# sanweiliti/RoHM

Hardware: AMD Instinct MI355X
Metric: denoised 145-frame clips/sec @1000 DDPM steps (higher is better)
Workload: dtype f32

## Files before the change

rohm_amd/csrc/encoder_chain.hip:

```cpp
#include <type_traits>
#include "common.h"
#include "gemm_sched.h"
#include "attention_tile.h"

namespace rohm {

typedef float f32x16c __attribute__((ext_vector_type(16)));

namespace chain {

constexpr int BM = 144, BK = kGemmBK, NRB = BM / 16;
constexpr int A_UNITS = BM * 8, A_ITERS = (A_UNITS + 255) / 256;
constexpr int kMaxBN = 384;
constexpr int kZone = 2 * (BM + kMaxBN) * BK;
constexpr int kLdsFloats = kZone + 512 + 4 * BM * 2;
constexpr int kSc1 = 16;

struct PhaseArgs {
    const float* A; int lda;
    const float* W; int ldw;
    float* C; int ldc;
    int K;
    const float* bias;
    const float* R; int ldr;
    const float* gamma; const float* beta; float eps; int ln_dim;
    int qcols; float qscale;
    int S; const float* tab; const float* tab0; int ldtab, ldtab0, tab_by_row;
    int m0, n0;
    float* row_stats; unsigned tag28; int tn, tiles_n;
    unsigned* err; unsigned xcc1; int fault;
};

__device__ __forceinline__ int head_row(int n0, int t) { return ((t % 96) >> 5) * 512 + n0 + (t / 96) * 32 + (t & 31); }

template <int BN, bool HEAD = false>
__device__ __forceinline__ void prefetch_w(const float* W, int ldw, int n0, float* smem, int tid, int wave_u) {
    constexpr int B_ITERS = BN * 8 / 256;
    float* Bs = smem + 2 * BM * BK;
#pragma unroll
    for (int buf = 0; buf < 2; ++buf)
#pragma unroll
        for (int i = 0; i < B_ITERS; ++i) {
            const int u = tid + i * 256;
            const int row = u >> 3;
            const int slot = (u & 7) ^ ((row >> 1) & 7);
            const float* src = W + (size_t)(HEAD ? head_row(n0, row) : n0 + row) * ldw + slot * 4 + buf * BK;
            __builtin_amdgcn_global_load_lds((const __attribute__((address_space(1))) void*)src,
                                             (__attribute__((address_space(3))) void*)(Bs + buf * (BN * BK) + (i * 256 + wave_u) * 4), 16, 0, 0);
        }
}

__device__ __forceinline__ void group_sync(unsigned long long* flags, int tn, int G, unsigned tag, unsigned xcc1, unsigned* err, int tid) {
    asm volatile("s_waitcnt vmcnt(0)" ::: "memory");
    __syncthreads();
    if (tid == 0) {
        flags[tn] = ((unsigned long long)xcc1 << 32) | tag;
        asm volatile("" ::: "memory");
    }
    if (tid < G && tid != tn) {
        for (int it = 0;; ++it) {
            const unsigned long long f = __hip_atomic_load(flags + tid, __ATOMIC_RELAXED, __HIP_MEMORY_SCOPE_AGENT);
            if ((unsigned)f == tag && (f >> 32) != 0ull) {
                if ((unsigned)(f >> 32) != xcc1) __hip_atomic_store(err, 2u, __ATOMIC_RELAXED, __HIP_MEMORY_SCOPE_AGENT);
                break;
            }
            __builtin_amdgcn_s_sleep(1);
            if ((it & 127) == 127 && __hip_atomic_load(err, __ATOMIC_RELAXED, __HIP_MEMORY_SCOPE_AGENT) != 0u) break;
            if (it > (1 << 19)) {
                __hip_atomic_store(err, 1u, __ATOMIC_RELAXED, __HIP_MEMORY_SCOPE_AGENT);
                break;
            }
        }
    }
    __syncthreads();
}

template <int BN, int EPI, bool PREF, bool SC1, bool REFETCH, bool HEAD = false, typename AfterLoop>
__device__ __forceinline__ void gemm_phase(const PhaseArgs& p, float* smem, const int tid, AfterLoop&& after_loop,
                                           AtQFrags<2>* q_out = nullptr) {
    static_assert(EPI == EPI_BIAS_RES_LN || EPI == EPI_BIAS_GELU || EPI == EPI_QKV || EPI == EPI_EMBED, "chain phases: LN tail, GELU, QKV, embed");
    static_assert(!HEAD || (EPI == EPI_QKV && BN == 3 * AT_DH), "the head-aligned tile is one head's q | k | v");
    constexpr int WN = BN / 4;
    constexpr int NCB = WN / 16;
    constexpr int B_ITERS = BN * 8 / 256;
    constexpr int PIECES = A_ITERS + B_ITERS;
    constexpr int AUX = SC1 ? kSc1 : 0;

    float* As = smem;
    float* Bs = smem + 2 * BM * BK;
    float* lds_dummy = smem + kZone;
    float* const zone = lds_dummy + 512;
    float* const colrow = HEAD ? smem + 2 * AT_TILE : zone;
    static_assert(!HEAD || 2 * AT_TILE + 512 <= AT_LDS_FLOATS, "head-aligned tile: the bias row overruns the stack's LDS");

    const int lane = tid & 63;
    const int wave = tid >> 6;
    const int li = lane & 15, lg = lane >> 4;
    const int wave_u = __builtin_amdgcn_readfirstlane(wave) * 64;
    const int m0 = p.m0, n0 = p.n0;

    const float* a_src[A_ITERS];
#pragma unroll
    for (int i = 0; i < A_ITERS; ++i) {
        const int u = tid + i * 256;
        const int row = (u < A_UNITS) ? (u >> 3) : 0;
        const int slot = (u & 7) ^ ((row >> 1) & 7);
        a_src[i] = p.A + (size_t)(m0 + row) * p.lda + slot * 4;
    }
    const float* b_src[B_ITERS];
#pragma unroll
    for (int i = 0; i < B_ITERS; ++i) {
        const int u = tid + i * 256;
        const int row = u >> 3;
        const int slot = (u & 7) ^ ((row >> 1) & 7);
        b_src[i] = p.W + (size_t)(HEAD ? head_row(n0, row) : n0 + row) * p.ldw + slot * 4;
    }
    auto dma_a = [&](int buf, int k0) {
#pragma unroll
        for (int piece = 0; piece < A_ITERS; ++piece) {
            float* dst = As + buf * (BM * BK) + (piece * 256 + wave_u) * 4;
            if (piece == A_ITERS - 1 && A_UNITS % 256 != 0)
                dst = (wave_u < A_UNITS - (A_ITERS - 1) * 256) ? dst : lds_dummy + (wave_u & 64) * 4;
            __builtin_amdgcn_global_load_lds((const __attribute__((address_space(1))) void*)(a_src[piece] + k0),
                                             (__attribute__((address_space(3))) void*)dst, 16, 0, AUX);
        }
    };
    auto dma_b = [&](int buf, int k0) {
#pragma unroll
        for (int i = 0; i < B_ITERS; ++i)
            __builtin_amdgcn_global_load_lds((const __attribute__((address_space(1))) void*)(b_src[i] + k0),
                                             (__attribute__((address_space(3))) void*)(Bs + buf * (BN * BK) + (i * 256 + wave_u) * 4), 16, 0, 0);
    };

    f32x4 acc16[NRB * NCB];
#pragma unroll
    for (int i = 0; i < NRB * NCB; ++i) acc16[i] = f32x4{0.f, 0.f, 0.f, 0.f};
    constexpr int READS = NRB + NCB;
    constexpr int MFMAS = 4 * NRB * NCB;
    struct Frag { f32x4 a[NRB]; f32x4 b[NCB]; };
    Frag f0, f1;
    auto read_frags = [&](Frag& f, int buf, int ks) {
        const float* as = As + buf * (BM * BK);
        const float* bs = Bs + buf * (BN * BK) + wave * WN * BK;
        const int slot = ks * 4 + lg;
#pragma unroll
        for (int c = 0; c < NCB; ++c) f.b[c] = *reinterpret_cast<const f32x4*>(bs + lds_off(c * 16 + li, slot));
#pragma unroll
        for (int r = 0; r < NRB; ++r) f.a[r] = *reinterpret_cast<const f32x4*>(as + lds_off(r * 16 + li, slot));
    };
    auto mma_half = [&](const Frag& f) {
#pragma unroll
        for (int r = 0; r < NRB; ++r)
#pragma unroll
            for (int c = 0; c < NCB; ++c)
#pragma unroll
                for (int j = 0; j < 4; ++j)
                    acc16[r * NCB + c] = __builtin_amdgcn_mfma_f32_16x16x4f32(f.b[c][j], f.a[r][j], acc16[r * NCB + c], 0, 0, 0);
    };

    const int nk = p.K / BK;
    constexpr bool COL_LDS = BN >= 384;
    if constexpr (!PREF) { dma_b(0, 0); dma_b(1, BK); }
    if constexpr (COL_LDS) {
        if (wave == 0) {
#pragma unroll
            for (int h = 0; h < 2; ++h) {
                const int unit = h * 64 + lane;
                const int t = (unit < BN / 4 ? unit : BN / 4 - 1) * 4;
                const float* src = HEAD ? p.bias + head_row(n0, t) : p.bias + n0 + t;
                __builtin_amdgcn_global_load_lds((const __attribute__((address_space(1))) void*)src,
                                                 (__attribute__((address_space(3))) void*)(colrow + h * 256), 16, 0, 0);
            }
        }
    }
    dma_a(0, 0);
    dma_a(1, BK);

    const int nw = n0 + wave * WN;
    struct ColOps { f32x4 bias, g4, b4; };
    constexpr bool RES = (EPI == EPI_BIAS_RES_LN);
    constexpr bool HAS_RES = RES || EPI == EPI_EMBED;
    constexpr bool PEEL = BN <= 256;
    constexpr bool EARLY = PEEL && !COL_LDS;
    const f32x4 zero4 = f32x4{0.f, 0.f, 0.f, 0.f};
    auto load_col = [&](int nb) __attribute__((always_inline)) {
        ColOps o{zero4, zero4, zero4};
        if constexpr (EPI == EPI_EMBED) {  }
        else if constexpr (COL_LDS) o.bias = *reinterpret_cast<const f32x4*>(colrow + (nb - n0));
        else o.bias = *reinterpret_cast<const f32x4*>(p.bias + nb);
        if constexpr (RES) {
            o.g4 = *reinterpret_cast<const f32x4*>(p.gamma + nb);
            o.b4 = *reinterpret_cast<const f32x4*>(p.beta + nb);
        }
        return o;
    };
    auto for_units = [&](auto&& fn) __attribute__((always_inline)) {
#pragma unroll
        for (int r = 0; r < NRB; ++r)
#pragma unroll
            for (int c = 0; c < NCB; ++c) fn(c * NRB + r, c, m0 + r * 16 + li, nw + c * 16 + lg * 4, acc16[r * NCB + c]);
    };
    ColOps col[NCB];
    f32x4 res[HAS_RES ? NCB * NRB : 1];
    auto request_ops = [&]() __attribute__((always_inline)) {
#pragma unroll
        for (int c = 0; c < NCB; ++c) col[c] = load_col(nw + c * 16 + lg * 4);
        if constexpr (RES)
            for_units([&](int i, int, int m, int nb, f32x4) __attribute__((always_inline)) {
                res[i] = *reinterpret_cast<const f32x4*>(p.R + (size_t)m * p.ldr + nb);
            });
        if constexpr (EPI == EPI_EMBED)
            for_units([&](int i, int, int m, int nb, f32x4) __attribute__((always_inline)) {
                const int bidx = m / p.S, tok = m % p.S;
                const float* tp = (tok == 0) ? p.tab0 + (size_t)bidx * p.ldtab0 + nb : p.tab + (size_t)(p.tab_by_row ? m : tok) * p.ldtab + nb;
                res[i] = *reinterpret_cast<const f32x4*>(tp);
            });
    };

    asm volatile("s_waitcnt vmcnt(%0)" ::"n"(A_ITERS) : "memory");
    __syncthreads();
    read_frags(f0, 0, 0);
    constexpr int NG = READS;
    constexpr int MF = (MFMAS + NG - 1) / NG;
    auto chunk = [&](int kc, auto last_tag, auto dma_tag) __attribute__((always_inline)) {
        constexpr bool LAST = decltype(last_tag)::value;
        constexpr bool DMA = decltype(dma_tag)::value;
        const int buf = kc & 1;
        if constexpr (LAST && EARLY) request_ops();
        read_frags(f1, buf, 1);
        mma_half(f0);
        SchedGroups<0, NG, MF, READS, 0, 0>::run();
        __builtin_amdgcn_sched_barrier(0);
        if constexpr (!LAST) {
            asm volatile("s_waitcnt vmcnt(0)" ::: "memory");
            __syncthreads();
            __builtin_amdgcn_sched_barrier(0);
            if constexpr (DMA) {
                const int kn = ((kc + 2 < nk) ? (kc + 2) : (nk - 1)) * BK;
                dma_a(buf, kn);
                dma_b(buf, kn);
            }
            read_frags(f0, buf ^ 1, 0);
            mma_half(f1);
            SchedGroups<0, NG, MF, READS, DMA ? PIECES : 0, 1>::run();
        } else {
            mma_half(f1);
        }
        __builtin_amdgcn_sched_barrier(0);
    };
    using DmaTail = std::integral_constant<bool, REFETCH>;
    if constexpr (PEEL) {
        for (int kc = 0; kc + 2 < nk; ++kc) chunk(kc, std::false_type{}, std::true_type{});
        chunk(nk - 2, std::false_type{}, DmaTail{});
        chunk(nk - 1, std::true_type{}, std::false_type{});
    } else {
        for (int kc = 0; kc + 2 < nk; ++kc) chunk(kc, std::false_type{}, std::true_type{});
        chunk(nk - 2, std::false_type{}, DmaTail{});
        chunk(nk - 1, std::false_type{}, DmaTail{});
    }
    asm volatile("s_waitcnt vmcnt(0)" ::: "memory");
    __syncthreads();
    after_loop();
    if constexpr (!EARLY) request_ops();

    if constexpr (EPI == EPI_BIAS_RES_LN) {
#pragma unroll
        for (int c = 0; c < NCB; ++c)
#pragma unroll
            for (int r = 0; r < NRB; ++r) {
                f32x4& a = acc16[r * NCB + c];
                const f32x4 rr = res[c * NRB + r];
#pragma unroll
                for (int q = 0; q < 4; ++q) a[q] = (a[q] + col[c].bias[q]) + rr[q];
            }
        typedef unsigned rohm_u2 __attribute__((ext_vector_type(2)));
        auto merge_swap = [](float& m, float& q2, float n, bool far) __attribute__((always_inline)) {
            rohm_u2 tm, tq;
            if (far) { tm = __builtin_amdgcn_permlane32_swap(__float_as_uint(m), __float_as_uint(m), false, false);
                       tq = __builtin_amdgcn_permlane32_swap(__float_as_uint(q2), __float_as_uint(q2), false, false); }
            else     { tm = __builtin_amdgcn_permlane16_swap(__float_as_uint(m), __float_as_uint(m), false, false);
                       tq = __builtin_amdgcn_permlane16_swap(__float_as_uint(q2), __float_as_uint(q2), false, false); }
            const float ma = __uint_as_float(tm[0]), mb = __uint_as_float(tm[1]);
            const float d = mb - ma;
            m = 0.5f * (ma + mb);
            q2 = (__uint_as_float(tq[0]) + __uint_as_float(tq[1])) + 0.5f * n * d * d;
        };
        float* const part = zone;
        constexpr float kLane = (float)(4 * NCB);
#pragma unroll
        for (int r = 0; r < NRB; ++r) {
            float sm = 0.f;
#pragma unroll
            for (int c = 0; c < NCB; ++c)
#pragma unroll
                for (int k = 0; k < 4; ++k) sm += acc16[r * NCB + c][k];
            float m = sm * (1.0f / kLane), q2 = 0.f;
#pragma unroll
            for (int c = 0; c < NCB; ++c)
#pragma unroll
                for (int k = 0; k < 4; ++k) { const float d = acc16[r * NCB + c][k] - m; q2 += d * d; }
            merge_swap(m, q2, kLane, true);
            merge_swap(m, q2, 2.0f * kLane, false);
            if (lg == 0) *reinterpret_cast<f32x2*>(part + (wave * BM + r * 16 + li) * 2) = f32x2{m, q2};
        }
        __syncthreads();
        const int tn = p.tn, tiles_n = p.tiles_n;
        const unsigned xcc1 = p.xcc1, ep28 = p.tag28;
        const unsigned tag = (ep28 << 4) | xcc1;
        float* const row_stats = p.row_stats;
        if (tid < BM) {
            auto merge = [](float ma, float qa, float mb, float qb, float n, float& m, float& q2) __attribute__((always_inline)) {
                const float d = mb - ma;
                m = 0.5f * (ma + mb);
                q2 = (qa + qb) + 0.5f * n * d * d;
            };
            f32x2 w4[4];
#pragma unroll
            for (int w = 0; w < 4; ++w) w4[w] = *reinterpret_cast<const f32x2*>(part + (w * BM + tid) * 2);
            float m01, q01, m23, q23, a, b;
            merge(w4[0][0], w4[0][1], w4[1][0], w4[1][1], (float)WN, m01, q01);
            merge(w4[2][0], w4[2][1], w4[3][0], w4[3][1], (float)WN, m23, q23);
            merge(m01, q01, m23, q23, 2.0f * (float)WN, a, b);
            const unsigned pub = (p.fault && tn == 0) ? (tag ^ 0x80000000u) : tag;
            *reinterpret_cast<f32x4*>(row_stats + ((size_t)tn * BM + tid) * 4) = f32x4{a, __uint_as_float(pub), b, __uint_as_float(pub)};
            float mk[8], qk[8];
            for (int it = 0;; ++it) {
                unsigned long long lo[8], hi[8];
#pragma unroll
                for (int k = 0; k < 8; ++k) {
                    lo[k] = hi[k] = 0ull;
                    if (k < tiles_n && k != tn) {
                        const unsigned long long* sp = reinterpret_cast<const unsigned long long*>(row_stats + ((size_t)k * BM + tid) * 4);
                        lo[k] = __hip_atomic_load(sp, __ATOMIC_RELAXED, __HIP_MEMORY_SCOPE_AGENT);
                        hi[k] = __hip_atomic_load(sp + 1, __ATOMIC_RELAXED, __HIP_MEMORY_SCOPE_AGENT);
                    }
                }
                bool ok = true, same_xcd = true;
#pragma unroll
                for (int k = 0; k < 8; ++k) {
                    mk[k] = 0.f; qk[k] = 0.f;
                    if (k >= tiles_n) continue;
                    if (k == tn) { mk[k] = a; qk[k] = b; continue; }
                    const unsigned tl = (unsigned)(lo[k] >> 32), th = (unsigned)(hi[k] >> 32);
                    ok = ok && (tl >> 4) == ep28 && (th >> 4) == ep28 && (tl & 15u) != 0u && (th & 15u) != 0u;
                    same_xcd = same_xcd && (tl & 15u) == xcc1 && (th & 15u) == xcc1;
                    mk[k] = __uint_as_float((unsigned)lo[k]);
                    qk[k] = __uint_as_float((unsigned)hi[k]);
                }
                if (ok) {
                    if (!same_xcd) __hip_atomic_store(p.err, 2u, __ATOMIC_RELAXED, __HIP_MEMORY_SCOPE_AGENT);
                    break;
                }
                __builtin_amdgcn_s_sleep(1);
                if ((it & 127) == 127 && __hip_atomic_load(p.err, __ATOMIC_RELAXED, __HIP_MEMORY_SCOPE_AGENT) != 0u) break;
                if (it > (1 << 19)) {
                    __hip_atomic_store(p.err, 1u, __ATOMIC_RELAXED, __HIP_MEMORY_SCOPE_AGENT);
                    break;
                }
            }
            constexpr float kT = (float)BN;
            if (tiles_n > 1) {
                merge(mk[0], qk[0], mk[1], qk[1], kT, mk[0], qk[0]);
                if (tiles_n > 2) merge(mk[2], qk[2], mk[3], qk[3], kT, mk[2], qk[2]);
                if (tiles_n > 4) { merge(mk[4], qk[4], mk[5], qk[5], kT, mk[4], qk[4]); merge(mk[6], qk[6], mk[7], qk[7], kT, mk[6], qk[6]); }
            }
            if (tiles_n > 2) {
                merge(mk[0], qk[0], mk[2], qk[2], 2.0f * kT, mk[0], qk[0]);
                if (tiles_n > 4) merge(mk[4], qk[4], mk[6], qk[6], 2.0f * kT, mk[4], qk[4]);
            }
            if (tiles_n > 4) merge(mk[0], qk[0], mk[4], qk[4], 4.0f * kT, mk[0], qk[0]);
            const float mu = mk[0];
            const float var = qk[0] / (float)p.ln_dim;
            *reinterpret_cast<f32x2*>(part + tid * 2) = f32x2{mu, 1.0f / sqrtf(var + p.eps)};
        }
        __syncthreads();
#pragma unroll
        for (int r = 0; r < NRB; ++r) {
            const f32x2 mrv = *reinterpret_cast<const f32x2*>(part + (r * 16 + li) * 2);
#pragma unroll
            for (int c = 0; c < NCB; ++c) {
                const f32x4 a = acc16[r * NCB + c];
                f32x4 v;
#pragma unroll
                for (int q = 0; q < 4; ++q) v[q] = (a[q] - mrv[0]) * mrv[1] * col[c].g4[q] + col[c].b4[q];
                *reinterpret_cast<f32x4*>(p.C + (size_t)(m0 + r * 16 + li) * p.ldc + nw + c * 16 + lg * 4) = v;
            }
        }
    } else if constexpr (HEAD) {
        float* const Ks = smem;
        float* const Vs = smem + AT_TILE;
        auto put = [&](float* img, int c) __attribute__((always_inline)) {
            const int u = wave * 8 + (c & 1) * 4 + lg;
#pragma unroll
            for (int r = 0; r < NRB; ++r) {
                const f32x4 a = acc16[r * NCB + c];
                f32x4 v;
#pragma unroll
                for (int q = 0; q < 4; ++q) v[q] = a[q] + col[c].bias[q];
                if (c < 2) {
#pragma unroll
                    for (int q = 0; q < 4; ++q) v[q] *= p.qscale;
                }
                *reinterpret_cast<f32x4*>(img + (r * 16 + li) * AT_DH + ((u ^ li) << 2)) = v;
            }
        };
        put(Vs, 0); put(Vs, 1);
        put(Ks, 2); put(Ks, 3);
        __syncthreads();
#pragma unroll
        for (int ks = 0; ks < 8; ++ks) {
            const int sw = ((ks * 4 + lg) ^ li) << 2;
#pragma unroll
            for (int ps = 0; ps < 2; ++ps) q_out->f[ps][ks] = *reinterpret_cast<const f32x4*>(Vs + ((ps * 4 + wave) * 16 + li) * AT_DH + sw);
            q_out->c[ks] = *reinterpret_cast<const f32x4*>(Vs + (8 * 16 + li) * AT_DH + sw);
        }
        __syncthreads();
        put(Vs, 4); put(Vs, 5);
    } else if constexpr (EPI == EPI_EMBED) {
        for_units([&](int i, int, int m, int nb, f32x4 a) __attribute__((always_inline)) {
            const int tok = m % p.S;
            f32x4 v;
#pragma unroll
            for (int q = 0; q < 4; ++q) v[q] = (tok == 0 ? 0.f : a[q]) + res[i][q];
            *reinterpret_cast<f32x4*>(p.C + (size_t)m * p.ldc + nb) = v;
        });
    } else {
        for_units([&](int, int cg, int m, int nb, f32x4 a) __attribute__((always_inline)) {
            f32x4 v;
#pragma unroll
            for (int q = 0; q < 4; ++q) v[q] = a[q] + col[cg].bias[q];
            if constexpr (EPI == EPI_BIAS_GELU) {
#pragma unroll
                for (int q = 0; q < 4; ++q) v[q] = gelu_erf(v[q]);
            }
            if constexpr (EPI == EPI_QKV) {
                if (nb < p.qcols) {
#pragma unroll
                    for (int q = 0; q < 4; ++q) v[q] *= p.qscale;
                }
            }
            *reinterpret_cast<f32x4*>(p.C + (size_t)m * p.ldc + nb) = v;
        });
    }
}

template <int G>
__device__ __forceinline__ void head_tail_phase(const StackParams& p, const int g, const int tn, float* smem, const int tid) {
    constexpr int NC_OWN = 16 / G;
    constexpr int NW = NC_OWN * 16 + 16;
    constexpr int NRMAX = (G == 4) ? 9 : 5;
    constexpr int W_UNITS = NW * 8, W_ITERS = (W_UNITS + 255) / 256;
    constexpr int PIECES = A_ITERS + W_ITERS;
    constexpr int kBuf = (BM + NW) * BK;
    static_assert(3 * kBuf <= kZone, "head phase: staging buffers overrun the zone");
    float* lds_dummy = smem + kZone;
    const int lane = tid & 63, li = lane & 15, lg = lane >> 4;
    const int wave = __builtin_amdgcn_readfirstlane(tid >> 6);
    const int wave_u = wave * 64;
    const int D = p.D, m0 = g * BM;
    int c_loc, r0, nr, e;
    if constexpr (G == 4) { c_loc = wave; r0 = 0; nr = 9; e = tn * 4 + wave; }
    else { c_loc = wave >> 1; r0 = (wave & 1) ? 5 : 0; nr = (wave & 1) ? 4 : 5; e = (wave & 1) ? tn * 2 + (wave >> 1) : 99; }
    const bool has_e = e < NRB;

    const float* a_src[A_ITERS];
#pragma unroll
    for (int i = 0; i < A_ITERS; ++i) {
        const int u = tid + i * 256;
        const int row = (u < A_UNITS) ? (u >> 3) : 0;
        const int slot = (u & 7) ^ ((row >> 1) & 7);
        a_src[i] = p.h + (size_t)(m0 + row) * D + slot * 4;
    }
    const float* w_src[W_ITERS];
#pragma unroll
    for (int i = 0; i < W_ITERS; ++i) {
        const int u = tid + i * 256;
        const int lrow = (u < W_UNITS) ? (u >> 3) : 0;
        const int slot = (u & 7) ^ ((lrow >> 1) & 7);
        const int grow = (lrow < NC_OWN * 16) ? tn * NC_OWN * 16 + lrow : 256 + (lrow - NC_OWN * 16);
        w_src[i] = p.t_out_w + (size_t)grow * D + slot * 4;
    }
    auto dma = [&](int buf, int k0) {
#pragma unroll
        for (int i = 0; i < A_ITERS; ++i) {
            float* dst = smem + buf * kBuf + (i * 256 + wave_u) * 4;
            if (i == A_ITERS - 1 && A_UNITS % 256 != 0)
                dst = (wave_u < A_UNITS - (A_ITERS - 1) * 256) ? dst : lds_dummy + (wave_u & 64) * 4;
            __builtin_amdgcn_global_load_lds((const __attribute__((address_space(1))) void*)(a_src[i] + k0),
                                             (__attribute__((address_space(3))) void*)dst, 16, 0, kSc1);
        }
#pragma unroll
        for (int i = 0; i < W_ITERS; ++i) {
            float* dst = smem + buf * kBuf + BM * BK + (i * 256 + wave_u) * 4;
            if (i == W_ITERS - 1 && W_UNITS % 256 != 0)
                dst = (wave_u < W_UNITS - (W_ITERS - 1) * 256) ? dst : lds_dummy + (wave_u & 64) * 4;
            __builtin_amdgcn_global_load_lds((const __attribute__((address_space(1))) void*)(w_src[i] + k0),
                                             (__attribute__((address_space(3))) void*)dst, 16, 0, 0);
        }
    };

    f32x4 acc[NRMAX], acc_e = f32x4{0.f, 0.f, 0.f, 0.f};
#pragma unroll
    for (int r = 0; r < NRMAX; ++r) acc[r] = f32x4{0.f, 0.f, 0.f, 0.f};
    const int nk = D / BK;
    dma(0, 0);
    dma(1, BK);

    typedef float f32x4u __attribute__((ext_vector_type(4), aligned(4)));
    const int C = p.t_C, T = p.t_T, traj = p.t_traj, S = BM;
    float* const x = p.t_x;
    const float* const nzp = p.t_noise;
    const size_t row_own = ((size_t)g * C + traj + (tn * NC_OWN + c_loc) * 16 + li) * T;
    const size_t row_sh = ((size_t)g * C + traj + 256 + li) * T;
    f32x4 xt[NRMAX], nz[NRMAX], xt_e = f32x4{0.f, 0.f, 0.f, 0.f}, nz_e = f32x4{0.f, 0.f, 0.f, 0.f};
#pragma unroll
    for (int r = 0; r < NRMAX; ++r) {
        xt[r] = nz[r] = f32x4{0.f, 0.f, 0.f, 0.f};
        if (r < nr) {
            const size_t idx = row_own + (size_t)((r0 + r) * 16 + 4 * lg) - 1;
            xt[r] = *reinterpret_cast<const f32x4u*>(x + idx);
            if (nzp) nz[r] = *reinterpret_cast<const f32x4u*>(nzp + idx);
        }
    }
    if (has_e) {
        const size_t idx = row_sh + (size_t)(e * 16 + 4 * lg) - 1;
        xt_e = *reinterpret_cast<const f32x4u*>(x + idx);
        if (nzp) nz_e = *reinterpret_cast<const f32x4u*>(nzp + idx);
    }
    const float bias_own = p.t_out_b[(tn * NC_OWN + c_loc) * 16 + li], bias_sh = p.t_out_b[256 + li];
    struct HFrag { f32x4 a[NRMAX]; f32x4 ae, w, wsh; };
    auto read_h = [&](HFrag& f, int b, int ks) __attribute__((always_inline)) {
        const float* as = smem + b * kBuf;
        const float* ws = as + BM * BK;
        const int slot = ks * 4 + lg;
        f.w = *reinterpret_cast<const f32x4*>(ws + lds_off(c_loc * 16 + li, slot));
#pragma unroll
        for (int r = 0; r < NRMAX; ++r)
            if (r < nr) f.a[r] = *reinterpret_cast<const f32x4*>(as + lds_off((r0 + r) * 16 + li, slot));
        if (has_e) {
            f.ae = *reinterpret_cast<const f32x4*>(as + lds_off(e * 16 + li, slot));
            f.wsh = *reinterpret_cast<const f32x4*>(ws + lds_off(NC_OWN * 16 + li, slot));
        }
    };
    auto mma_h = [&](const HFrag& f) __attribute__((always_inline)) {
#pragma unroll
        for (int r = 0; r < NRMAX; ++r)
            if (r < nr) {
#pragma unroll
                for (int j = 0; j < 4; ++j) acc[r] = __builtin_amdgcn_mfma_f32_16x16x4f32(f.a[r][j], f.w[j], acc[r], 0, 0, 0);
            }
        if (has_e) {
#pragma unroll
            for (int j = 0; j < 4; ++j) acc_e = __builtin_amdgcn_mfma_f32_16x16x4f32(f.ae[j], f.wsh[j], acc_e, 0, 0, 0);
        }
    };
    HFrag f0, f1;
    f0.ae = f0.wsh = f1.ae = f1.wsh = f32x4{0.f, 0.f, 0.f, 0.f};
#pragma unroll
    for (int r = 0; r < NRMAX; ++r) f0.a[r] = f1.a[r] = f32x4{0.f, 0.f, 0.f, 0.f};
    asm volatile("s_waitcnt vmcnt(0)" ::: "memory");
    __syncthreads();
    read_h(f0, 0, 0);
    int buf = 0;
    for (int kc = 0; kc < nk; ++kc) {
        AT_WAIT_LGKM0();
        __builtin_amdgcn_sched_barrier(0);
        read_h(f1, buf, 1);
        __builtin_amdgcn_sched_barrier(0);
        mma_h(f0);
        __builtin_amdgcn_sched_barrier(0);
        const int nbuf = buf == 2 ? 0 : buf + 1;
        if (kc + 1 < nk) {
            asm volatile("s_waitcnt vmcnt(0)" ::: "memory");
            __syncthreads();
            __builtin_amdgcn_sched_barrier(0);
            if (kc + 2 < nk) dma(buf >= 1 ? buf - 1 : 2, (kc + 2) * BK);
            AT_WAIT_LGKM0();
            __builtin_amdgcn_sched_barrier(0);
            read_h(f0, nbuf, 0);
            __builtin_amdgcn_sched_barrier(0);
        } else {
            AT_WAIT_LGKM0();
        }
        mma_h(f1);
        __builtin_amdgcn_sched_barrier(0);
        buf = nbuf;
    }

    const float c1 = p.t_c1, c2 = p.t_c2, sg = p.t_sigma;
    float* const x0o = p.t_x0;
    float* const apk = p.t_apack;
    auto emit = [&](int rblk, size_t row, int ch, float bias, const f32x4& a, const f32x4& xv, const f32x4& nv) __attribute__((always_inline)) {
        const int tok0 = rblk * 16 + 4 * lg;
        f32x4 val, o;
#pragma unroll
        for (int v = 0; v < 4; ++v) {
            val[v] = a[v] + bias;
            o[v] = c1 * val[v] + c2 * xv[v];
            if (nzp) o[v] += sg * nv[v];
        }
        const size_t idx = row + (size_t)tok0 - 1;
        if (tok0 != 0) {
            if (x0o) *reinterpret_cast<f32x4u*>(x0o + idx) = val;
            *reinterpret_cast<f32x4u*>(x + idx) = o;
        } else {
#pragma unroll
            for (int v = 1; v < 4; ++v) {
                if (x0o) x0o[idx + v] = val[v];
                x[idx + v] = o[v];
            }
        }
        if (apk) {
            float* const d = apk + ((size_t)g * S + tok0) * p.t_lda + traj + ch;
#pragma unroll
            for (int v = 0; v < 4; ++v)
                if (tok0 + v != 0) d[(size_t)v * p.t_lda] = o[v];
        }
    };
#pragma unroll
    for (int r = 0; r < NRMAX; ++r)
        if (r < nr) emit(r0 + r, row_own, (tn * NC_OWN + c_loc) * 16 + li, bias_own, acc[r], xt[r], nz[r]);
    if (has_e) emit(e, row_sh, 256 + li, bias_sh, acc_e, xt_e, nz_e);
    for (int i = tn * 256 + tid; i < traj * T; i += G * 256) {
        const int ch = i / T, t = i - ch * T;
        const size_t idx = ((size_t)g * C + ch) * T + t;
        const float val = p.t_cond[idx];
        if (x0o) x0o[idx] = val;
        float o = c1 * val + c2 * x[idx];
        if (nzp) o += sg * nzp[idx];
        x[idx] = o;
        if (apk) apk[((size_t)g * S + t + 1) * p.t_lda + ch] = o;
    }
}

}

template <int G>
__global__ __launch_bounds__(256) void encoder_chain_kernel(ChainParams p) {
    using namespace chain;
    constexpr int BNL = 512 / G, BNF = 1024 / G, BNQ = 1536 / G;
    extern __shared__ __attribute__((aligned(16))) float smem[];
    const int tid = threadIdx.x;
    const int wave_u = __builtin_amdgcn_readfirstlane(tid >> 6) * 64;
    const int x = blockIdx.x % kNumXCD, j = blockIdx.x / kNumXCD;
    const int g = (j / G) * kNumXCD + x, tn = j % G;
    if (g >= p.tiles_m) return;
    const unsigned xcc1 = 1u + (unsigned)__builtin_amdgcn_s_getreg((3 << 11) | 20);
    const unsigned ep = p.epoch + 64u * *p.xln_pass;
    if (tid == 0) p.xln_xcc[g * 8 + tn] = xcc1;
    unsigned long long* const flags = p.flags + (size_t)g * 9 * 5 * 8;

    PhaseArgs a{};
    a.m0 = g * BM; a.err = p.xln_err; a.xcc1 = xcc1; a.tn = tn; a.tiles_n = G;
    a.row_stats = p.xln_stats + ((size_t)g * G * BM) * 4;
    a.eps = p.ln_eps; a.ln_dim = p.D;

    a.A = p.ctx; a.lda = p.D; a.W = p.out_w; a.ldw = p.D; a.C = p.y; a.ldc = p.D; a.K = p.D; a.bias = p.out_b;
    a.R = p.h; a.ldr = p.D; a.gamma = p.n1_w; a.beta = p.n1_b; a.n0 = tn * BNL; a.tag28 = ep & 0x0fffffffu; a.fault = p.fault & 1;
    gemm_phase<BNL, EPI_BIAS_RES_LN, false, false, G == 8>(a, smem, tid, [&]() { prefetch_w<BNF>(p.l1_w, p.D, tn * BNF, smem, tid, wave_u); });
    group_sync(flags, tn, G, ep, xcc1, p.xln_err, tid);

    a.A = p.y; a.lda = p.D; a.W = p.l1_w; a.ldw = p.D; a.C = p.ff; a.ldc = p.F; a.K = p.D; a.bias = p.l1_b; a.n0 = tn * BNF;
    gemm_phase<BNF, EPI_BIAS_GELU, true, true, G == 8>(a, smem, tid, [&]() { prefetch_w<BNL>(p.l2_w, p.F, tn * BNL, smem, tid, wave_u); });
    group_sync(flags + 8, tn, G, ep, xcc1, p.xln_err, tid);

    a.A = p.ff; a.lda = p.F; a.W = p.l2_w; a.ldw = p.F; a.C = p.h; a.ldc = p.D; a.K = p.F; a.bias = p.l2_b;
    a.R = p.y; a.ldr = p.D; a.gamma = p.n2_w; a.beta = p.n2_b; a.n0 = tn * BNL; a.tag28 = (ep + 1u) & 0x0fffffffu; a.fault = (p.fault >> 1) & 1;
    gemm_phase<BNL, EPI_BIAS_RES_LN, true, true, G == 8>(a, smem, tid, [&]() { if (p.qkv) prefetch_w<BNQ>(p.in_w, p.D, tn * BNQ, smem, tid, wave_u); });
    if (p.qkv == nullptr) return;
    group_sync(flags + 16, tn, G, ep, xcc1, p.xln_err, tid);

    a.A = p.h; a.lda = p.D; a.W = p.in_w; a.ldw = p.D; a.C = p.qkv; a.ldc = 3 * p.D; a.K = p.D; a.bias = p.in_b; a.n0 = tn * BNQ;
    a.qcols = p.D; a.qscale = p.qscale;
    gemm_phase<BNQ, EPI_QKV, true, true, G == 8>(a, smem, tid, []() {});
}

template <int G>
__global__ __launch_bounds__(256) void encoder_stack_kernel(StackParams p) {
    using namespace chain;
    constexpr int BNL = 512 / G, BNF = 1024 / G, BNQ = 1536 / G;
    extern __shared__ __attribute__((aligned(16))) float smem[];
    const int tid0 = threadIdx.x;
    const int x = blockIdx.x % kNumXCD, j = blockIdx.x / kNumXCD;
    const int g = (j / G) * kNumXCD + x, tn = j % G;
    if (g >= p.tiles_m) return;
    const unsigned xcc1 = 1u + (unsigned)__builtin_amdgcn_s_getreg((3 << 11) | 20);
    const unsigned ep = p.epoch + 64u * (*p.xln_pass + p.pass_add);
    if (tid0 == 0) p.xln_xcc[g * 8 + tn] = xcc1;

    PhaseArgs a{};
    a.m0 = g * BM; a.err = p.xln_err; a.xcc1 = xcc1; a.tn = tn; a.tiles_n = G;
    a.row_stats = p.xln_stats + ((size_t)g * G * BM) * 4;
    a.eps = p.ln_eps; a.ln_dim = p.D;
    a.qcols = p.D; a.qscale = p.qscale;
    constexpr bool HEAD = G == 4;
    auto n0q = [&]() __attribute__((always_inline)) { return HEAD ? tn * AT_DH : tn * BNQ; };
    AtQFrags<2> qh;
    unsigned long long* const tl = p.timeline ? p.timeline + (size_t)blockIdx.x * kStackTimelineLayers * kStackTimelineStamps : nullptr;
    auto stamp = [&](int layer, int k) __attribute__((always_inline)) {
        if (tl != nullptr && threadIdx.x == 0) tl[layer * kStackTimelineStamps + k] = __builtin_amdgcn_s_memrealtime();
    };
    auto attend = [&](int l, int tid) __attribute__((always_inline)) {
        unsigned long long* const fl = p.flags + ((size_t)g * 9 + l) * 5 * 8;
        stamp(l, 0);
        if (l > 0) {
            if constexpr (HEAD) __syncthreads();
            else group_sync(fl, tn, G, ep, xcc1, p.xln_err, tid);
        }
        stamp(l, 1);
        if constexpr (HEAD)
            attention_item<4, 0, kSc1, 2, true>(p.qkv, p.ctx, p.n_head, g * p.n_head + tn, 0, AT_NB, smem, tid, &qh);
        else attention_item<4, 0, kSc1, 1>(p.qkv, p.ctx, p.n_head, g * p.n_head + (tn >> 1), (tn & 1) ? 5 : 0, (tn & 1) ? 4 : 5, smem, tid);
        stamp(l, 2);
        group_sync(fl + 8, tn, G, ep, xcc1, p.xln_err, tid);
        stamp(l, 3);
    };
    {
    int tid = tid0;
    asm volatile("" : "+v"(tid));
    const int wave_u = __builtin_amdgcn_readfirstlane(tid >> 6) * 64;
    unsigned long long* const fl = p.flags + ((size_t)g * 9 + 8) * 5 * 8;
    a.A = p.apack; a.lda = p.lda_pack; a.W = p.w_embed; a.ldw = p.ldw_embed; a.C = p.h; a.ldc = p.D; a.K = p.k_embed; a.n0 = tn * BNL;
    a.S = p.S; a.tab = p.tab; a.tab0 = p.tab0; a.ldtab = p.ldtab; a.ldtab0 = p.ldtab0; a.tab_by_row = p.tab_by_row;
    stamp(8, 0);
    gemm_phase<BNL, EPI_EMBED, false, false, G == 8>(a, smem, tid, [&]() { prefetch_w<BNQ, HEAD>(p.layer[0].in_w, p.D, n0q(), smem, tid, wave_u); });
    stamp(8, 1);
    group_sync(fl, tn, G, ep, xcc1, p.xln_err, tid);
    stamp(8, 2);
    a.A = p.h; a.lda = p.D; a.W = p.layer[0].in_w; a.ldw = p.D; a.C = p.qkv; a.ldc = 3 * p.D; a.K = p.D; a.bias = p.layer[0].in_b;
    a.n0 = n0q();
    gemm_phase<BNQ, EPI_QKV, true, true, G == 8, HEAD>(a, smem, tid, []() {}, &qh);
    stamp(8, 3);
    if constexpr (HEAD) __syncthreads();
    else group_sync(fl + 8, tn, G, ep, xcc1, p.xln_err, tid);
    stamp(8, 4);
    if constexpr (HEAD) attend(0, tid);
    }
#pragma unroll 1
    for (int l = 0; l < p.L; ++l) {
        int tid = tid0;
        asm volatile("" : "+v"(tid));
        const int wave_u = __builtin_amdgcn_readfirstlane(tid >> 6) * 64;
        const StackLayerW& w = p.layer[l];
        unsigned long long* const fl = p.flags + ((size_t)g * 9 + l) * 5 * 8;
        if constexpr (!HEAD) attend(l, tid);

        a.A = p.ctx; a.lda = p.D; a.W = w.out_w; a.ldw = p.D; a.C = p.y; a.ldc = p.D; a.K = p.D; a.bias = w.out_b;
        a.R = p.h; a.ldr = p.D; a.gamma = w.n1_w; a.beta = w.n1_b; a.n0 = tn * BNL; a.tag28 = (ep + 4u * l) & 0x0fffffffu;
        a.fault = (l == 0) ? (p.fault & 1) : 0;
        gemm_phase<BNL, EPI_BIAS_RES_LN, false, true, G == 8>(a, smem, tid, [&]() { prefetch_w<BNF>(w.l1_w, p.D, tn * BNF, smem, tid, wave_u); });
        stamp(l, 4);
        group_sync(fl + 16, tn, G, ep, xcc1, p.xln_err, tid);
        stamp(l, 5);

        a.A = p.y; a.lda = p.D; a.W = w.l1_w; a.ldw = p.D; a.C = p.ff; a.ldc = p.F; a.K = p.D; a.bias = w.l1_b; a.n0 = tn * BNF;
        gemm_phase<BNF, EPI_BIAS_GELU, true, true, G == 8>(a, smem, tid, [&]() { prefetch_w<BNL>(w.l2_w, p.F, tn * BNL, smem, tid, wave_u); });
        stamp(l, 6);
        group_sync(fl + 24, tn, G, ep, xcc1, p.xln_err, tid);
        stamp(l, 7);

        const bool more = l + 1 < p.L;
        a.A = p.ff; a.lda = p.F; a.W = w.l2_w; a.ldw = p.F; a.C = p.h; a.ldc = p.D; a.K = p.F; a.bias = w.l2_b;
        a.R = p.y; a.ldr = p.D; a.gamma = w.n2_w; a.beta = w.n2_b; a.n0 = tn * BNL; a.tag28 = (ep + 4u * l + 1u) & 0x0fffffffu;
        a.fault = (l == 0) ? ((p.fault >> 1) & 1) : 0;
        gemm_phase<BNL, EPI_BIAS_RES_LN, true, true, G == 8>(a, smem, tid, [&]() { if (more) prefetch_w<BNQ, HEAD>(p.layer[l + 1].in_w, p.D, n0q(), smem, tid, wave_u); });
        stamp(l, 8);
        if (!more) {
            if (p.tail) {
                group_sync(fl + 32, tn, G, ep, xcc1, p.xln_err, tid);
                stamp(l, 9);
                head_tail_phase<G>(p, g, tn, smem, tid);
                stamp(l, 10);
                if (p.t_pass_ctr != nullptr && blockIdx.x == 0 && threadIdx.x == 0) p.t_pass_ctr[1] = p.pass_add + 1u;
            }
            break;
        }
        group_sync(fl + 32, tn, G, ep, xcc1, p.xln_err, tid);
        stamp(l, 9);

        a.A = p.h; a.lda = p.D; a.W = p.layer[l + 1].in_w; a.ldw = p.D; a.C = p.qkv; a.ldc = 3 * p.D; a.K = p.D; a.bias = p.layer[l + 1].in_b;
        a.n0 = n0q();
        gemm_phase<BNQ, EPI_QKV, true, true, G == 8, HEAD>(a, smem, tid, []() {}, &qh);
        stamp(l, 10);
        if constexpr (HEAD) attend(l + 1, tid);
    }
}

int launch_encoder_stack(const StackParams& p, hipStream_t s) {
    const int G = encoder_chain_parts(p.M, p.D, p.F);
    ROHM_ARG_CHECK(G != 0 && p.n_head == 4 && p.L >= 1 && p.L <= 8, "encoder_stack: shape (M %d, D %d, F %d, %d heads, %d layers) has no stack form",
                   p.M, p.D, p.F, p.n_head, p.L);
    ROHM_ARG_CHECK(p.h && p.y && p.ff && p.qkv && p.ctx && p.xln_stats && p.xln_err && p.xln_pass && p.xln_xcc && p.flags, "encoder_stack: null operand");
    ROHM_ARG_CHECK(p.apack && p.w_embed && p.tab && p.tab0 && p.S == chain::BM && p.k_embed >= 2 * chain::BK && p.k_embed % chain::BK == 0 &&
                       p.lda_pack % 4 == 0 && p.ldw_embed % 4 == 0 && p.ldtab % 4 == 0 && p.ldtab0 % 4 == 0,
                   "encoder_stack: bad operands of the leading embed phase");
    StackParams q = p;
    q.tiles_m = p.M / chain::BM;
    const int groups8 = (q.tiles_m + kNumXCD - 1) / kNumXCD * kNumXCD;
    ROHM_ARG_CHECK(!p.tail || (p.D == 512 && p.t_out_w && p.t_out_b && p.t_x && p.t_cond && p.t_C - p.t_traj == 272 &&
                               p.t_T == chain::BM - 1 && p.t_traj > 0 && (!p.t_apack || p.t_lda >= p.t_C)),
                   "encoder_stack: the closing head / update / pack phase needs whole 144-token clips, d_model 512 and 272 predicted channels");
    constexpr int kFloats = AT_LDS_FLOATS > chain::kLdsFloats ? AT_LDS_FLOATS : chain::kLdsFloats;
    const size_t lds = (size_t)kFloats * sizeof(float);
    static bool attr_set[64][2] = {};
    int dev = 0;
    ROHM_HIP_CHECK(hipGetDevice(&dev));
    if (dev < 64 && !attr_set[dev][G == 8]) {
        if (G == 4) ROHM_HIP_CHECK(hipFuncSetAttribute(reinterpret_cast<const void*>(&encoder_stack_kernel<4>), hipFuncAttributeMaxDynamicSharedMemorySize, (int)lds));
        else ROHM_HIP_CHECK(hipFuncSetAttribute(reinterpret_cast<const void*>(&encoder_stack_kernel<8>), hipFuncAttributeMaxDynamicSharedMemorySize, (int)lds));
        attr_set[dev][G == 8] = true;
    }
    const double MM = (double)p.M, D = p.D, F = p.F, L = p.L;
    const double flops = L * (4.0 * 144.0 * 128.0 * MM * p.n_head + 2.0 * MM * (D * D + 2.0 * D * F)) + L * 2.0 * MM * 3.0 * D * D +
                         2.0 * MM * D * p.k_embed;
    const double bytes = 4.0 * (L * (MM * (3.0 * D + D + 4.0 * D + 2.0 * F + D) + D * D + 2.0 * D * F) + (L - 1.0) * (MM * 3.0 * D + 3.0 * D * D));
    const double tail_flops = p.tail ? 2.0 * MM * D * (p.t_C - p.t_traj) : 0.0;
    prof::Scope ps(p.tail ? "gemm_stack_tail" : "gemm_stack", flops + tail_flops, bytes, s);
    if (G == 4) hipLaunchKernelGGL(encoder_stack_kernel<4>, dim3(groups8 * 4), dim3(256), lds, s, q);
    else hipLaunchKernelGGL(encoder_stack_kernel<8>, dim3(groups8 * 8), dim3(256), lds, s, q);
    ROHM_LAUNCH_CHECK();
    return ROHM_OK;
}

int encoder_chain_parts(int M, int D, int F) {
    if (D != 512 || F != 1024 || M <= 0 || M % chain::BM != 0) return 0;
    const int tm = M / chain::BM;
    return tm >= 48 ? 4 : 8;
}

bool encoder_chain_pays(int B) {
    if (B <= 0) return false;
    if (B < 48) return B > 24 && B <= 32;
    if (B <= 64) return true;
    const int wgs = (B + kNumXCD - 1) / kNumXCD * kNumXCD * 4, rounds = (wgs + 255) / 256;
    return 4 * B * 100 >= 93 * rounds * 256;
}

size_t encoder_chain_flag_bytes(int M) { return (size_t)((M + chain::BM - 1) / chain::BM) * 9 * 5 * 8 * sizeof(unsigned long long); }

int launch_encoder_chain(const ChainParams& p, hipStream_t s) {
    const int G = encoder_chain_parts(p.M, p.D, p.F);
    ROHM_ARG_CHECK(G != 0, "encoder_chain: shape (M %d, D %d, F %d) has no chain form", p.M, p.D, p.F);
    ROHM_ARG_CHECK(p.ctx && p.h && p.y && p.ff && p.out_w && p.out_b && p.n1_w && p.n1_b && p.l1_w && p.l1_b && p.l2_w && p.l2_b &&
                       p.n2_w && p.n2_b && p.xln_stats && p.xln_err && p.xln_pass && p.xln_xcc && p.flags && (!p.qkv || (p.in_w && p.in_b)),
                   "encoder_chain: null operand");
    ChainParams q = p;
    q.tiles_m = p.M / chain::BM;
    const int groups8 = (q.tiles_m + kNumXCD - 1) / kNumXCD * kNumXCD;
    const size_t lds = (size_t)chain::kLdsFloats * sizeof(float);
    static bool attr_set[64][2] = {};
    int dev = 0;
    ROHM_HIP_CHECK(hipGetDevice(&dev));
    if (dev < 64 && !attr_set[dev][G == 8]) {
        if (G == 4) ROHM_HIP_CHECK(hipFuncSetAttribute(reinterpret_cast<const void*>(&encoder_chain_kernel<4>), hipFuncAttributeMaxDynamicSharedMemorySize, (int)lds));
        else ROHM_HIP_CHECK(hipFuncSetAttribute(reinterpret_cast<const void*>(&encoder_chain_kernel<8>), hipFuncAttributeMaxDynamicSharedMemorySize, (int)lds));
        attr_set[dev][G == 8] = true;
    }
    const double MM = (double)p.M, D = p.D, F = p.F;
    const double flops = 2.0 * MM * (D * D + 2.0 * D * F + (p.qkv ? 3.0 * D * D : 0.0));
    const double bytes = 4.0 * (MM * (4.0 * D + 2.0 * F + D + (p.qkv ? 3.0 * D : 0.0)) + D * D + 2.0 * D * F + (p.qkv ? 3.0 * D * D : 0.0));
    prof::Scope ps(p.qkv ? "gemm_chain" : "gemm_chain_last", flops, bytes, s);
    if (G == 4) hipLaunchKernelGGL(encoder_chain_kernel<4>, dim3(groups8 * 4), dim3(256), lds, s, q);
    else hipLaunchKernelGGL(encoder_chain_kernel<8>, dim3(groups8 * 8), dim3(256), lds, s, q);
    ROHM_LAUNCH_CHECK();
    return ROHM_OK;
}

}
```

Baseline: 23.39.

## Interleave bias-residual-LayerNorm row stats with final k-chunk MFMAs

```diff
diff --git a/rohm_amd/csrc/encoder_chain.hip b/rohm_amd/csrc/encoder_chain.hip
--- a/rohm_amd/csrc/encoder_chain.hip
+++ b/rohm_amd/csrc/encoder_chain.hip
@@ -222,10 +222,93 @@
     read_frags(f0, 0, 0);
     constexpr int NG = READS;
     constexpr int MF = (MFMAS + NG - 1) / NG;
+    constexpr bool DRIP = PEEL && !HEAD && EPI == EPI_BIAS_RES_LN;
+    constexpr int kFirst = NCB >= 2 ? 1 : 2;
+    constexpr int kAhead = NCB >= 2 ? 1 : 2;
+    constexpr int kDripValu = 6;
+    typedef unsigned rohm_u2 __attribute__((ext_vector_type(2)));
+    auto merge_swap = [](float& m, float& q2, float n, bool far) __attribute__((always_inline)) {
+        rohm_u2 tm, tq;
+        if (far) { tm = __builtin_amdgcn_permlane32_swap(__float_as_uint(m), __float_as_uint(m), false, false);
+                   tq = __builtin_amdgcn_permlane32_swap(__float_as_uint(q2), __float_as_uint(q2), false, false); }
+        else     { tm = __builtin_amdgcn_permlane16_swap(__float_as_uint(m), __float_as_uint(m), false, false);
+                   tq = __builtin_amdgcn_permlane16_swap(__float_as_uint(q2), __float_as_uint(q2), false, false); }
+        const float ma = __uint_as_float(tm[0]), mb = __uint_as_float(tm[1]);
+        const float d = mb - ma;
+        m = 0.5f * (ma + mb);
+        q2 = (__uint_as_float(tq[0]) + __uint_as_float(tq[1])) + 0.5f * n * d * d;
+    };
+    float* const part = zone;
+    auto request_res_row = [&](int r) __attribute__((always_inline)) {
+#pragma unroll
+        for (int c = 0; c < NCB; ++c)
+            res[c * NRB + r] = *reinterpret_cast<const f32x4*>(p.R + (size_t)(m0 + r * 16 + li) * p.ldr + nw + c * 16 + lg * 4);
+    };
+    auto ln_row = [&](int r) __attribute__((always_inline)) {
+        constexpr float kLane = (float)(4 * NCB);
+#pragma unroll
+        for (int c = 0; c < NCB; ++c) {
+            f32x4& a = acc16[r * NCB + c];
+            const f32x4 rr = res[c * NRB + r];
+#pragma unroll
+            for (int q = 0; q < 4; ++q) a[q] = (a[q] + col[c].bias[q]) + rr[q];
+        }
+        float sm = 0.f;
+#pragma unroll
+        for (int c = 0; c < NCB; ++c)
+#pragma unroll
+            for (int k = 0; k < 4; ++k) sm += acc16[r * NCB + c][k];
+        float m = sm * (1.0f / kLane), q2 = 0.f;
+#pragma unroll
+        for (int c = 0; c < NCB; ++c)
+#pragma unroll
+            for (int k = 0; k < 4; ++k) { const float d = acc16[r * NCB + c][k] - m; q2 += d * d; }
+        merge_swap(m, q2, kLane, true);
+        merge_swap(m, q2, 2.0f * kLane, false);
+        if (lg == 0) *reinterpret_cast<f32x2*>(part + (wave * BM + r * 16 + li) * 2) = f32x2{m, q2};
+    };
+    auto mma_cols = [&](const Frag& f, int r, int c0, int nc) __attribute__((always_inline)) {
+#pragma unroll
+        for (int c = c0; c < c0 + nc; ++c)
+#pragma unroll
+            for (int j = 0; j < 4; ++j)
+                acc16[r * NCB + c] = __builtin_amdgcn_mfma_f32_16x16x4f32(f.b[c][j], f.a[r][j], acc16[r * NCB + c], 0, 0, 0);
+    };
     auto chunk = [&](int kc, auto last_tag, auto dma_tag) __attribute__((always_inline)) {
         constexpr bool LAST = decltype(last_tag)::value;
         constexpr bool DMA = decltype(dma_tag)::value;
         const int buf = kc & 1;
+        if constexpr (LAST && DRIP) {
+#pragma unroll
+            for (int c = 0; c < NCB; ++c) col[c] = load_col(nw + c * 16 + lg * 4);
+#pragma unroll
+            for (int r = 0; r <= kAhead; ++r) request_res_row(r);
+            __builtin_amdgcn_sched_barrier(0);
+            const float* as1 = As + buf * (BM * BK);
+            const float* bs1 = Bs + buf * (BN * BK) + wave * WN * BK;
+            const int slot1 = 4 + lg;
+#pragma unroll
+            for (int c = 0; c < NCB; ++c) f1.b[c] = *reinterpret_cast<const f32x4*>(bs1 + lds_off(c * 16 + li, slot1));
+#pragma unroll
+            for (int r = 0; r < kFirst; ++r) f1.a[r] = *reinterpret_cast<const f32x4*>(as1 + lds_off(r * 16 + li, slot1));
+            mma_cols(f0, 0, 0, NCB);
+            mma_cols(f1, 0, 0, NCB);
+            SchedGroups<0, 4 * NCB, 1, NCB + kFirst, 0, 0>::run();
+            __builtin_amdgcn_sched_group_barrier(0x008, 4 * NCB, 0);
+            __builtin_amdgcn_sched_barrier(0);
+#pragma unroll
+            for (int r = 1; r < NRB; ++r) {
+                if (r + kFirst - 1 < NRB) f1.a[r + kFirst - 1] = *reinterpret_cast<const f32x4*>(as1 + lds_off((r + kFirst - 1) * 16 + li, slot1));
+                if (r + kAhead < NRB) request_res_row(r + kAhead);
+                mma_cols(f0, r, 0, NCB);
+                mma_cols(f1, r, 0, NCB);
+                ln_row(r - 1);
+                SchedGroups<0, 1, 1, 1, NCB, 0, kDripValu>::run();
+                SchedGroups<0, 8 * NCB - 1, 1, 0, 0, 0, kDripValu>::run();
+                __builtin_amdgcn_sched_barrier(0);
+            }
+            return;
+        }
         if constexpr (LAST && EARLY) request_ops();
         read_frags(f1, buf, 1);
         mma_half(f0);
@@ -265,44 +348,7 @@
 
     if constexpr (EPI == EPI_BIAS_RES_LN) {
 #pragma unroll
-        for (int c = 0; c < NCB; ++c)
-#pragma unroll
-            for (int r = 0; r < NRB; ++r) {
-                f32x4& a = acc16[r * NCB + c];
-                const f32x4 rr = res[c * NRB + r];
-#pragma unroll
-                for (int q = 0; q < 4; ++q) a[q] = (a[q] + col[c].bias[q]) + rr[q];
-            }
-        typedef unsigned rohm_u2 __attribute__((ext_vector_type(2)));
-        auto merge_swap = [](float& m, float& q2, float n, bool far) __attribute__((always_inline)) {
-            rohm_u2 tm, tq;
-            if (far) { tm = __builtin_amdgcn_permlane32_swap(__float_as_uint(m), __float_as_uint(m), false, false);
-                       tq = __builtin_amdgcn_permlane32_swap(__float_as_uint(q2), __float_as_uint(q2), false, false); }
-            else     { tm = __builtin_amdgcn_permlane16_swap(__float_as_uint(m), __float_as_uint(m), false, false);
-                       tq = __builtin_amdgcn_permlane16_swap(__float_as_uint(q2), __float_as_uint(q2), false, false); }
-            const float ma = __uint_as_float(tm[0]), mb = __uint_as_float(tm[1]);
-            const float d = mb - ma;
-            m = 0.5f * (ma + mb);
-            q2 = (__uint_as_float(tq[0]) + __uint_as_float(tq[1])) + 0.5f * n * d * d;
-        };
-        float* const part = zone;
-        constexpr float kLane = (float)(4 * NCB);
-#pragma unroll
-        for (int r = 0; r < NRB; ++r) {
-            float sm = 0.f;
-#pragma unroll
-            for (int c = 0; c < NCB; ++c)
-#pragma unroll
-                for (int k = 0; k < 4; ++k) sm += acc16[r * NCB + c][k];
-            float m = sm * (1.0f / kLane), q2 = 0.f;
-#pragma unroll
-            for (int c = 0; c < NCB; ++c)
-#pragma unroll
-                for (int k = 0; k < 4; ++k) { const float d = acc16[r * NCB + c][k] - m; q2 += d * d; }
-            merge_swap(m, q2, kLane, true);
-            merge_swap(m, q2, 2.0f * kLane, false);
-            if (lg == 0) *reinterpret_cast<f32x2*>(part + (wave * BM + r * 16 + li) * 2) = f32x2{m, q2};
-        }
+        for (int r = DRIP ? NRB - 1 : 0; r < NRB; ++r) ln_row(r);
         __syncthreads();
         const int tn = p.tn, tiles_n = p.tiles_n;
         const unsigned xcc1 = p.xcc1, ep28 = p.tag28;
```

New measurement: 23.46, median of 6. Within noise of the previous version (+0.3%).
